# sleep3r/Diffusion-Handwriting-Generation.pytorch

Measured on AMD Instinct MI355X. Metric: stroke-points/sec reverse-sampled (T=60, L=488), higher is better.
Workload: dtype bf16; 1 GPU; configs[1]: batch=64 prompts/GPU, T=60, L=488, Lt=30, d_model=128/192/256, num_layers=2, diffusion_mode=new, random-init weights; global_batch=64, seq_len=488, parallelism=batch-shard x1 (no collectives)

## Files before the change

diffusion-handwriting-generation.pytorch_amd/csrc/dhw_api.cpp:

```cpp
#include <hip/hip_runtime.h>

#include <algorithm>
#include <cmath>
#include <cstdarg>
#include <cstdio>
#include <cstdlib>
#include <cstring>
#include <map>
#include <string>
#include <vector>

#include "../../include/dhw.h"
#include "abi_guard.h"
#include "xcd_swizzle.h"
#include "../../include/dhw_debug.h"
#include "dhw_kernels.h"
#include "persist.h"

namespace {

constexpr int SIG = 32, SIG_HID = 2048, VOCAB = 73, STYLE_CH = 256;
constexpr int SLACK_ROWS = 64;

ErrBuf g_err;
// ... 164 lines not shown

  float *sg_w1, *sg_b1, *sg_w2, *sg_b2, *in_w, *in_b, *out_w, *out_b, *pen_w, *pen_b, *emb;

  ConvBlockW enc1, enc2, enc4, dec3, dec2, dec1;
  std::vector<EncLayerW> el;
  void *w_sf1, *w_sf3, *w_q8, *w_kv8, *w_d8, *w_tf1, *w_tf3, *w_attd, *w_sk1, *w_sk2, *w_sk3;
  float *b_sf1, *b_sf3, *b_q8, *b_kv8, *b_d8, *b_tf1, *b_tf3, *b_attd, *b_sk1, *b_sk2, *b_sk3;
  int f_ts1, f_ts2, f_ts3, f_ts4;

  std::vector<Workspace> ws;
  int nstreams = 1;
  int nstreams_alloc = 1;
  hipStream_t sub_streams[MAX_STREAMS] = {};
  std::vector<TapSlot> taps;
  std::vector<std::string> el_name;
  int lpadT = 0, lpadS = 0, lpadX[3] = {0, 0, 0};

  bool prof = false;
  std::vector<std::string> prof_labels;
  std::vector<ProfRec> prof_recs;
  std::vector<ProfAgg> prof_agg;

  bool use_graph = true;
  int teach_every = 0;
  const float* teach_reset = nullptr;
  float* teach_capture = nullptr;
  bool fuse_heads = true;
  bool plane = true;
  bool fuse_up = true;
  bool chain = true;
  bool fuse = true;
  bool fuse_text = true;
  int text_pairs = 0;
  std::map<std::vector<uint64_t>, hipGraphExec_t> graphs;
  int64_t* d_text_stage = nullptr;
  float* d_style_stage = nullptr;
  float* d_out_stage = nullptr;
  float* d_noise_stage = nullptr;
  size_t noise_stage_cap = 0;
  uint64_t* d_seed = nullptr;

  bool persist = false;
  int persist_grid = 0;
  unsigned* d_step_sync = nullptr;
  size_t step_sync_words = 0;
  unsigned* h_step_err = nullptr;
  unsigned* d_step_err = nullptr;
  struct StepPlans { StepPlan* dev = nullptr; bool ok = false; };
  unsigned long long* d_step_trace = nullptr;
  std::map<std::vector<uint64_t>, StepPlans> plans;

  int last_B = 0, last_L = 0, last_Lt = 0;
};

namespace {

int fail(dhw_handle* h, int code, const char* fmt, ...) noexcept {
  va_list ap;
  va_start(ap, fmt);
  g_err.vsetf(fmt, ap);
  va_end(ap);
  if (h) h->err.set(g_err.c_str());
  return code;
}

#define DHW_GUARD(h, fn, R, ...) \
// ... 757 lines not shown
    GemmParams p = gp_base(c, c.S5, 4 * c2);
    p.seg[0] = GemmSeg{WS(c, sty_in), h->w_sf1, STYLE_CH, 1, 1};
    p.bias0 = h->b_sf1;
    p.silu_out = 1;
    p.out = WS(c, sty_h);
    run_gemm(c, "style.ffn1", p);
  }
  {
    GemmParams p = gp_base(c, c.S5, dt);
    p.seg[0] = GemmSeg{WS(c, sty_h), h->w_sf3, 4 * c2, 1, 0};
    p.bias0 = h->b_sf3;
    p.ln = 1;
    p.out = WS(c, sty_n);
    run_gemm(c, "style.ffn2_ln", p);
  }
  RUN_SMALL(c, "embed_ln", launch_embed_ln(h->prec, text, c.B * c.Lt, h->emb, dt, true_width(h, dt), VOCAB, WS(c, t_n), c.st));
}

void text_style_dynamic(Ctx& c) {
  dhw_handle* h = c.h;
  const int c2 = h->dims.c2, dt = 2 * c2;
  const float* g = c.film;
  const float* bt = c.film + h->film_tot;
  const int in_B = c.in_B ? c.in_B : c.B;
  if (h->fuse && h->fuse_text && textside_supported(h->prec, c.Lt, c.S5, dt)) {
    TextStyleParams q{};
    q.n = c.B; q.in_B = in_B; q.Lt = c.Lt; q.S5 = c.S5;
    q.sty_n = WS(c, sty_n); q.t_n = WS(c, t_n);
    q.film = c.film; q.film_bs = c.film_bs; q.film_div = c.film_div; q.film_tot = h->film_tot;
    q.f1 = h->f_ts1; q.f2 = h->f_ts2; q.f3 = h->f_ts3; q.f4 = h->f_ts4;
    q.w_q8 = h->w_q8; q.w_kv8 = h->w_kv8; q.w_d8 = h->w_d8; q.w_tf1 = h->w_tf1; q.w_tf3 = h->w_tf3;
    q.b_q8 = h->b_q8; q.b_kv8 = h->b_kv8; q.b_d8 = h->b_d8; q.b_tf1 = h->b_tf1; q.b_tf3 = h->b_tf3;
    q.text_out = TS(c, text_out);
    if (!c.err) {
      const double n = c.B, ddt = dt;
      Launch l(h, c.st, "ts.fused", n * (2.0 * c.S5 * ddt * 2 * ddt + 2.0 * c.Lt * ddt * ddt * 2 + 4.0 * c.Lt * c.S5 * ddt + 2.0 * c.Lt * ddt * 2 * ddt * 2),
               n * c.Lt * ddt * h->es + (double)in_B * (c.S5 + c.Lt) * ddt * h->es + 8.0 * ddt * ddt * h->es);
      hipError_t e = launch_text_style(h->prec, q, c.st);
      if (e != hipSuccess) c.err = fail(h, DHW_ERR_HIP, "text_style fused: %s", hipGetErrorString(e));
    }
    if (!c.planeT) tap(c, TAP_TS, TS(c, text_out), c.Lt, dt);
    for (size_t i = 0; i < h->el.size() && !c.err; ++i) {
      const EncLayerW& w = h->el[i];
      TextLayerParams t{};
      t.n = c.B; t.Lt = c.Lt; t.d = w.d;
      t.text_out = TS(c, text_out);
      t.w_td = w.w_td; t.b_td = w.b_td;
      t.film = c.film; t.film_bs = c.film_bs; t.film_div = c.film_div; t.film_tot = h->film_tot; t.f0 = w.f0;
      t.w_kv = w.w_kv1; t.b_kv = w.b_kv1; t.pb_k1 = w.pb_k1;
      t.k1 = ELT(c, (int)i, k1); t.vt1 = ELT(c, (int)i, vt1); t.lpadT = h->lpadT;
      if (c.err) break;
      t.pairs = h->text_pairs;
      const double n = c.B, dd = w.d;
      Launch l(h, c.st, "enc.text_fused", n * c.Lt * (2.0 * dt * dd + 4.0 * dd * dd), n * c.Lt * (dt + 2.0 * dd) * h->es + (dt * dd + 2.0 * dd * dd) * h->es);
      hipError_t e = launch_text_layer(h->prec, t, c.st);
      if (e != hipSuccess) c.err = fail(h, DHW_ERR_HIP, "text layer %s: %s", h->el_name[i].c_str(), hipGetErrorString(e));
    }
    return;
  }
  RUN_SMALL(c, "film.style", launch_film_apply(h->prec, WS(c, sty_n), in_B, c.B, c.S5, dt, g + h->f_ts1, bt + h->f_ts1, c.film_bs, c.film_div, TS(c, s1), c.st));
  RUN_SMALL(c, "film.text", launch_film_apply(h->prec, WS(c, t_n), in_B, c.B, c.Lt, dt, g + h->f_ts2, bt + h->f_ts2, c.film_bs, c.film_div, TS(c, t1), c.st));
  {
    GemmParams p = gp_text(c, c.Lt, dt);
    p.seg[0] = GemmSeg{TS(c, t1), h->w_q8, dt, 1, 0};
    p.bias0 = h->b_q8;
    p.out = TS(c, q8);
    run_gemm(c, "ts.q", p);
  }
  {
    GemmParams p = gp_base(c, c.S5, 2 * dt);
    p.seg[0] = GemmSeg{TS(c, s1), h->w_kv8, dt, 1, 0};
    p.bias0 = h->b_kv8;
    p.n_store = dt;
    p.out = TS(c, k8);
    p.vt = TS(c, vt8);
    p.vt_lpad = h->lpadS;
    run_gemm(c, "ts.kv", p);
  }
  {
    AttnParams a{};
    a.Q = TS(c, q8); a.ldq = dt;
    a.K = TS(c, k8); a.ldk = dt; a.koff = 0;
    a.Vt = TS(c, vt8); a.lpad = h->lpadS;
    a.out = TS(c, a8); a.ldo = dt;
    a.B = c.B; a.H = 8; a.D = dt / 8; a.Lq = c.Lt; a.Lk = c.S5;
    run_attn(c, "attn.text_style", a);
// ... 236 lines not shown
    h->dims.c2 = 192;
    h->padded = d.c2 != 192;
    h->device = device;
    h->prec = d.precision == DHW_PREC_F32 ? PREC_F32 : PREC_BF16;
    h->es = h->prec == PREC_F32 ? 4 : 2;
    h->spec = build_spec(d.num_layers, d.c1, d.c2, d.c3);
    h->pspec = build_spec(d.num_layers, d.c1, h->dims.c2, d.c3);
    for (size_t i = 0; i < h->spec.size(); ++i) h->key_index[h->spec[i].key] = (int)i;
    h->host_w.resize(h->spec.size());
    h->loaded.assign(h->spec.size(), 0);
    build_film_layout(h);
    build_names(h);
    if (hipSetDevice(device) != hipSuccess) return fail(nullptr, DHW_ERR_HIP, "hipSetDevice failed");
    {
      const char* e = getenv("DHW_STREAMS");
      if (e && atoi(e) >= 1) h->nstreams = std::min(atoi(e), MAX_STREAMS);
      h->nstreams = std::max(1, std::min(h->nstreams, d.max_B));
      h->nstreams_alloc = h->nstreams;
    }
    int rc = alloc_shared(h);
    h->ws.resize(h->nstreams);
    for (int i = 0; !rc && i < h->nstreams; ++i)
      if (!(rc = alloc_workspace(h, h->ws[i], i == 0 ? d.max_B : (d.max_B + h->nstreams - 1) / h->nstreams))) rc = verify_workspace(h, h->ws[i]);
    for (int i = 1; !rc && i < h->nstreams; ++i)
      if (hipStreamCreateWithFlags(&h->sub_streams[i], hipStreamNonBlocking) != hipSuccess) rc = fail(h, DHW_ERR_HIP, "stream create failed");
    if (const char* e = getenv("DHW_FUSE")) h->fuse = atoi(e) != 0;
    if (const char* e = getenv("DHW_PLANE")) h->plane = atoi(e) != 0;
    if (const char* e = getenv("DHW_FUSE_TEXT")) h->fuse_text = atoi(e) != 0;
    if (const char* e = getenv("DHW_FUSE_HEADS")) h->fuse_heads = atoi(e) != 0;
    if (const char* e = getenv("DHW_FUSE_UP")) h->fuse_up = atoi(e) != 0;
    if (const char* e = getenv("DHW_CHAIN")) h->chain = atoi(e) != 0;
    if (const char* e = getenv("DHW_PERSIST")) h->persist = atoi(e) != 0;
    if (const char* e = getenv("DHW_TEXT_PAIRS")) h->text_pairs = atoi(e) == 1 ? 1 : atoi(e) == 2 ? 2 : 0;
    if (h->padded) h->fuse = false;
    if (!rc && h->prec == PREC_BF16 && h->persist) {
      hipDeviceProp_t prop;
      if (hipGetDeviceProperties(&prop, device) != hipSuccess || persist_init() != hipSuccess) rc = fail(h, DHW_ERR_HIP, "persistent kernel setup failed: %s", hipGetErrorString(hipGetLastError()));
      else {
        h->persist_grid = prop.multiProcessorCount;
        if (hipHostMalloc((void**)&h->h_step_err, 64, hipHostMallocMapped) != hipSuccess || hipHostGetDevicePointer((void**)&h->d_step_err, h->h_step_err, 0) != hipSuccess)
          rc = fail(h, DHW_ERR_HIP, "host-mapped error word: %s", hipGetErrorString(hipGetLastError()));
        else *h->h_step_err = 0;
      }
    }
    if (!rc && enclayer_init() != hipSuccess) rc = fail(h, DHW_ERR_HIP, "kernel attribute setup failed: %s", hipGetErrorString(hipGetLastError()));
    if (!rc && convblock_init() != hipSuccess) rc = fail(h, DHW_ERR_HIP, "kernel attribute setup failed: %s", hipGetErrorString(hipGetLastError()));
    if (!rc && textside_init() != hipSuccess) rc = fail(h, DHW_ERR_HIP, "kernel attribute setup failed: %s", hipGetErrorString(hipGetLastError()));
    if (!rc && gemm_init() != hipSuccess) rc = fail(h, DHW_ERR_HIP, "kernel attribute setup failed: %s", hipGetErrorString(hipGetLastError()));
    if (rc) { ErrBuf keep = h->err; g_err = keep; return rc; }
    hold.p = nullptr;
    *out = h;
    return 0;
  });
}

void dhw_destroy(dhw_handle* h) {
  if (!h) return;
  try {
    destroy_impl(h);
  } catch (...) {
  }
}

}

namespace {
// ... 657 lines not shown
```

diffusion-handwriting-generation.pytorch_amd/csrc/dhw_kernels.h:

```cpp
#pragma once
#include <hip/hip_runtime.h>
#include <stdint.h>

enum { PREC_BF16 = 0, PREC_F32 = 1 };

struct GemmSeg {
  const void* A;
  const void* W;
  int C;
  int taps;
  int silu;
};

struct GemmParams {
  GemmSeg seg[2];
  int nseg;
  int B, L;
  int N;
  int n_store;
  const float* bias0;
  const float* bias1;
  const float* posb;
  int posb_cols;
  const float* gam;
// ... 117 lines not shown
hipError_t launch_randn_init(float* xt, long rows, int L, const uint64_t* seed_ptr, int sample_off, hipStream_t st, int iter = -1);
hipError_t launch_set_seed(uint64_t* seed_ptr, uint64_t seed, int64_t first_sample, hipStream_t st);
hipError_t gemm_init();

hipError_t launch_style_stem(int prec, const float* img, int B, int H, int W, const float* w, const float* bias, int Cp,
                             void* out, hipStream_t st);
hipError_t launch_style_dw(int prec, const void* in, int B, int H, int W, int stride, const float* w, const float* bias,
                           int Cp, void* out, hipStream_t st);
hipError_t launch_style_pool(int prec, const void* in, int B, int H, int W, int C, int NB, float* out, hipStream_t st);

struct TextStyleParams {
  int n;
  int in_B;
  int Lt, S5;
  const void* sty_n;
  const void* t_n;
  const float* film; long film_bs; int film_div; int film_tot;
  int f1, f2, f3, f4;
  const void *w_q8, *w_kv8, *w_d8, *w_tf1, *w_tf3;
  const float *b_q8, *b_kv8, *b_d8, *b_tf1, *b_tf3;
  void* text_out;
};
struct TextLayerParams {
  int n, Lt, d;
  const void* text_out;
  const void* w_td; const float* b_td;
  const float* film; long film_bs; int film_div; int film_tot; int f0;
  const void* w_kv; const float* b_kv;
  const float* pb_k1;
  void* k1;
  void* vt1; int lpadT;
  int pairs;
};
bool textside_supported(int prec, int Lt, int S5, int dt);
hipError_t launch_text_style(int prec, const TextStyleParams& p, hipStream_t st);
hipError_t launch_text_layer(int prec, const TextLayerParams& p, hipStream_t st);
hipError_t textside_init();

hipError_t launch_perturb(const float* x, const float* eps, const float* alphas, int B, int L, float* out, hipStream_t st);
hipError_t launch_loss(const float* eps, const float* pred, const float* pen, const float* pen_pred, const float* alphas, int B, int L,
                       float* out3, float* d_pred, float* d_pen, hipStream_t st);
hipError_t launch_sqnorm(const float* g, long n, float* out, hipStream_t st);
hipError_t launch_adam(float* p, const float* g, float* m, float* v, long n, float lr, float b1, float b2, float eps, float wd, int step,
                       const float* sqnorm, float max_norm, hipStream_t st);
hipError_t launch_film_silu_fwd(const float* u, const float* film, long film_bs, int goff, int boff, int B, int L, int C, float* a, float* h, hipStream_t st);
hipError_t launch_film_bwd(const float* d, const float* a, const float* u, const float* film, long film_bs, int goff, int B, int L, int C, int act,
                           float* du, float* dfilm, long dfilm_bs, int dgoff, int dboff, hipStream_t st);
hipError_t launch_silu_bwd_add(const float* d_sx, const float* x, long n, float* dx, hipStream_t st);
hipError_t launch_silu_fwd(const float* x, long n, float* out, hipStream_t st);
hipError_t launch_add(const float* a, const float* b, long n, float* out, hipStream_t st);
hipError_t launch_colsum(const float* dy, long rows, int C, float* db, hipStream_t st);
hipError_t launch_wgrad(const float* dy, const float* x, int B, int L, int Cout, int Cin, int taps, float* dw, hipStream_t st);
hipError_t launch_film_linear_bwd(const float* dfilm, const float* sigma, const float* wcat, int B, int cols, float* dw, float* db, float* dsigma, hipStream_t st);

struct OpGemm {
  const float* A; long sam, sak, sazo, sazi; int a_shift, a_tap_shift;
  const float* B; long sbk, sbn, sbzo, sbzi, sbt; int b_shift, b_z_shift;
  float* C; long scm, scn, sczo, sczi;
  int M, N, K, nzo, nzi, lr, taps;
  const float* bias; float alpha; int accumulate, bf16;
  const float* dsilu_of;
  float* act_out;
  const float* addend;
  float* rowsum;
  unsigned long long* stamps;
  const float* film_g = nullptr; const float* film_b = nullptr; long film_ps = 0; int film_rows = 1, film_act = 0; float* film_out = nullptr; const float* film_add = nullptr;
};
// ... 31 lines not shown
```

diffusion-handwriting-generation.pytorch_amd/csrc/textside.hip:

```cpp
#include <algorithm>
#include "enc_a_core.h"

namespace {

template <typename T, int D, int NK>
DHW_DEV void attn_once(
    const Frag<T> (&qf)[2], const char* kt, int SK, const char* vt, int SV, int Lk, f32x4 (&o)[D / 16]) {
  constexpr int DT = D / 16, NPF = (NK + 1) / 2;
  const int lane = threadIdx.x & 63, g = lane >> 4;
  const float scale = rsqrtf((float)D);
  f32x4 s[NK];
#pragma unroll
  for (int t = 0; t < NK; ++t) {
    s[t] = (f32x4){0, 0, 0, 0};
#pragma unroll
    for (int c = 0; c < 2; ++c) {
      const int d = 32 * c + 8 * g;
      const Frag<T> kf = d < D ? frag_load(reinterpret_cast<const T*>(kt + t * 16 * SK) + d) : frag_zero<T>();
      mma32(s[t], kf, qf[c]);
    }
  }
  float mx = -INFINITY;
#pragma unroll
  for (int t = 0; t < NK; ++t)
// ... 49 lines not shown
  }
};

template <typename T, int KMAX>
DHW_DEV void stage_film_384(char* dst, int S, const T* src, int rows_valid, int rows_tile, const float* gam, const float* bet, int tid) {
  static_assert(sizeof(T) == 2, "bf16 only");
  if (tid >= 480) return;
  const int cc = tid % 48, r0 = tid / 48;
  const f32x4 g0 = *reinterpret_cast<const f32x4*>(gam + cc * 8), g1 = *reinterpret_cast<const f32x4*>(gam + cc * 8 + 4);
  const f32x4 b0 = *reinterpret_cast<const f32x4*>(bet + cc * 8), b1 = *reinterpret_cast<const f32x4*>(bet + cc * 8 + 4);
  uint4 v[KMAX];
#pragma unroll
  for (int k = 0; k < KMAX; ++k) {
    const int r = r0 + 10 * k;
    v[k] = make_uint4(0, 0, 0, 0);
    if (r < rows_valid) v[k] = *reinterpret_cast<const uint4*>(src + (size_t)r * 384 + cc * 8);
  }
#pragma unroll
  for (int k = 0; k < KMAX; ++k) {
    const int r = r0 + 10 * k;
    if (r >= rows_tile) continue;
    if (r < rows_valid) {
      T* e = reinterpret_cast<T*>(&v[k]);
#pragma unroll
      for (int i = 0; i < 4; ++i) {
        e[i] = from_f<T>(to_f(e[i]) * g0[i] + b0[i]);
        e[4 + i] = from_f<T>(to_f(e[4 + i]) * g1[i] + b1[i]);
      }
    }
    *reinterpret_cast<uint4*>(dst + r * S + cc * 16) = v[k];
  }
}

template <typename T>
__global__ __launch_bounds__(512) __attribute__((amdgpu_waves_per_eu(2, 2))) void text_style_kernel(const TextStyleParams p) {
  constexpr int ES = sizeof(T), DM = 384, BM = 32, SM = 80, D = 48, KC = DM / 32;
  constexpr int NT = DM / 8 / 16, MT = BM / 16, MTS = SM / 16;
  constexpr int S = tile_stride<T>(DM), SVT = SM * ES + 16;
  extern __shared__ __attribute__((aligned(16))) char smem[];
  char* RS = smem;
  char* RV = RS + SM * S;
  char* RT = RV + DM * SVT;
  float* red = reinterpret_cast<float*>(RT + BM * S);
  const int tid = threadIdx.x, lane = tid & 63, wave = tid >> 6, l15 = lane & 15, g = lane >> 4;
  const int pair = blockIdx.x;
  const int bs = pair % p.in_B;
  const float* gam = p.film + (long)(pair / p.film_div) * p.film_bs;
  const float* bet = gam + p.film_tot;
  const int ntile0 = wave * NT, n0 = ntile0 * 16 + 4 * g;
  const size_t wlane = ((size_t)ntile0 * KC * 64 + lane) * 8;
  const T* sty = reinterpret_cast<const T*>(p.sty_n) + (size_t)bs * p.S5 * DM;
  const T* tn = reinterpret_cast<const T*>(p.t_n) + (size_t)bs * p.Lt * DM;
  const char* sop = RS + l15 * S + g * 8 * ES;
  const char* top = RT + l15 * S + g * 8 * ES;

  WRing<T, NT> ring;
#ifndef DHW_TEXT_SPREAD
#define DHW_TEXT_SPREAD 1
#endif
  constexpr bool TSPREAD = DHW_TEXT_SPREAD != 0;
  constexpr int FC = WRing<T, NT>::template fill_chunks<KC>(), FQ = (FC + 3) / 4;
  EpiParams<NT> ep;

  stage_film_384<T, 8>(RS, S, sty, p.S5, SM, gam + p.f1, bet + p.f1, tid);
  stage_film_384<T, 4>(RT, S, tn, p.Lt, BM, gam + p.f2, bet + p.f2, tid);
  ring.template fill_s<KC>(reinterpret_cast<const T*>(p.w_kv8) + (size_t)DM * DM + wlane);
  ep.load_bias(p.b_kv8 + DM, n0);
  lds_barrier();

  {
    f32x4 acc[NT][MTS];
    acc_zero(acc);
    ring.template run_s<MTS, KC>(acc, sop, S, KC);
    if constexpr (TSPREAD) ring.template fill_begin<KC>(reinterpret_cast<const T*>(p.w_kv8) + wlane);
    else ring.template fill_s<KC>(reinterpret_cast<const T*>(p.w_kv8) + wlane);
#pragma unroll
    for (int i = 0; i < NT; ++i) {
      if constexpr (TSPREAD) {
        if (i == 0) ring.template fill_range<KC, 0, FQ>();
        else if (i == 1) ring.template fill_range<KC, FQ, 2 * FQ>();
        else if (i == 2) ring.template fill_range<KC, 2 * FQ, 3 * FQ>();
      }
#pragma unroll
      for (int j = 0; j < MTS; ++j) {
        const int key = j * 16 + l15;
        const f32x4 v = acc[i][j] + ep.bias[i];
#pragma unroll
        for (int k = 0; k < 4; ++k) *reinterpret_cast<T*>(RV + (n0 + 16 * i + k) * SVT + key * ES) = from_f<T>(key < p.S5 ? v[k] : 0.f);
      }
    }
    if constexpr (TSPREAD) { static_assert(NT == 3, "three channel tiles per wave"); ring.template fill_range<KC, 3 * FQ, FC>(); }
    ep.load_bias(p.b_kv8, n0);
// ... 101 lines not shown
        else if (i == 1) ring.template fill_range<KC, FQ, 2 * FQ>();
        else if (i == 2) ring.template fill_range<KC, 2 * FQ, 3 * FQ>();
      }
#pragma unroll
      for (int j = 0; j < MT; ++j) {
        f32x4 v = acc[i][j] + ep.bias[i];
#pragma unroll
        for (int k = 0; k < 4; ++k) v[k] = silu_t<T>(v[k]);
        store4(reinterpret_cast<T*>(HID + (j * 16 + l15) * S) + n0 + 16 * i, v);
      }
    }
    if constexpr (TSPREAD) ring.template fill_range<KC, 3 * FQ, FC>();
    lds_barrier();
    ring.template run_s<MT, KC>(acc2, hop, S, KC);
    if (hh == 0) {
      ring.template fill_s<KC>(reinterpret_cast<const T*>(p.w_tf1) + (size_t)DM * DM + wlane);
      lds_barrier();
    }
  }
  ep.load(p.b_tf3, gam + p.f4, bet + p.f4, n0);
#pragma unroll
  for (int i = 0; i < NT; ++i)
#pragma unroll
    for (int j = 0; j < MT; ++j) acc2[i][j] += ep.bias[i];
  ln_rows<T, MT, NT, 8, BM>(acc2, red, wave, 0, lane, DM);
#pragma unroll
  for (int i = 0; i < NT; ++i)
#pragma unroll
    for (int j = 0; j < MT; ++j) store4(reinterpret_cast<T*>(T2 + (j * 16 + l15) * S) + n0 + 16 * i, acc2[i][j] * ep.gam[i] + ep.bet[i]);
  lds_barrier();
  tile_copy_out<T>(T2, S, reinterpret_cast<T*>(p.text_out) + (size_t)pair * p.Lt * DM, DM, p.Lt, DM, tid, 512);
}

template <typename T, int DMO, int PAIRS>
__global__ __launch_bounds__(512) __attribute__((amdgpu_waves_per_eu(4 / PAIRS, 4 / PAIRS))) void text_layer_kernel(const TextLayerParams p) {
  constexpr int OCC = 2 / PAIRS;
  constexpr int ES = sizeof(T), DI = 384, BM = 32 * PAIRS, KCI = DI / 32, KCO = DMO / 32;
  constexpr int WN = (DMO % 128 == 0) ? 8 : 6, NT = DMO / WN / 16, MT = BM / 16;
  constexpr int SI = tile_stride<T>(DI), SO = tile_stride<T>(DMO);
  extern __shared__ __attribute__((aligned(16))) char smem[];
  char* XS = smem;
  char* TL = XS + BM * SI;
  float* red = reinterpret_cast<float*>(TL + BM * SO);
  const int tid = threadIdx.x, lane = tid & 63, wave = tid >> 6, l15 = lane & 15, g = lane >> 4;
#ifndef DHW_TEXT_SPREAD
#define DHW_TEXT_SPREAD 1
#endif
  constexpr bool TSPREAD = DHW_TEXT_SPREAD != 0;
  const int pair = blockIdx.x * PAIRS;
  const int npair = min(PAIRS, p.n - pair);
  const float* gam = p.film + (long)(pair / p.film_div) * p.film_bs;
  const float* bet = gam + p.film_tot;
  const bool act = WN == 8 || wave < WN;
  const int wn = act ? wave : 0, ntile0 = wn * NT, n0 = ntile0 * 16 + 4 * g;

  WRing<T, NT, 24 / OCC> ring;
  constexpr int FCO = WRing<T, NT, 24 / OCC>::template fill_chunks<KCO>(), FQO = (FCO + 3) / 4;
  EpiParams<NT> ep;
  {
    const T* src = reinterpret_cast<const T*>(p.text_out) + (size_t)pair * p.Lt * DI;
    constexpr int cpr = DI * ES / 16, NU = BM * cpr / 512;
    static_assert(BM * cpr % 512 == 0, "staging chunks per thread");
    uint4 v[NU];
#pragma unroll
    for (int u = 0; u < NU; ++u) {
      const int id = tid + u * 512, r = id / cpr, cc = id - r * cpr, pr = r >> 5, rr = r & 31;
      const bool ok = pr < npair && rr < p.Lt;
      v[u] = *reinterpret_cast<const uint4*>(src + (ok ? (size_t)pr * p.Lt + rr : (size_t)0) * DI + cc * (16 / ES));
    }
#pragma unroll
    for (int u = 0; u < NU; ++u) {
      const int id = tid + u * 512, r = id / cpr, cc = id - r * cpr, pr = r >> 5, rr = r & 31;
      const bool ok = pr < npair && rr < p.Lt;
      T* e = reinterpret_cast<T*>(&v[u]);
#pragma unroll
      for (int i = 0; i < 16 / ES; ++i) e[i] = from_f<T>(silu_t<T>(to_f(e[i])));
      *reinterpret_cast<uint4*>(XS + r * SI + cc * 16) = ok ? v[u] : make_uint4(0, 0, 0, 0);
    }
  }
  if (act) {
    ring.template fill_s<KCI>(reinterpret_cast<const T*>(p.w_td) + ((size_t)ntile0 * KCI * 64 + lane) * 8);
    ep.load(p.b_td, gam + p.f0, bet + p.f0, n0);
  }
  lds_barrier();

  {
    f32x4 acc[NT][MT];
    acc_zero(acc);
    if (act) {
      ring.template run_s<MT, KCI>(acc, XS + l15 * SI + g * 8 * ES, SI, KCI);
      if constexpr (TSPREAD) { ring.template fill_begin<KCO>(reinterpret_cast<const T*>(p.w_kv) + ((size_t)ntile0 * KCO * 64 + lane) * 8); ring.template fill_range<KCO, 0, FQO>(); }
      else ring.template fill_s<KCO>(reinterpret_cast<const T*>(p.w_kv) + ((size_t)ntile0 * KCO * 64 + lane) * 8);
#pragma unroll
      for (int i = 0; i < NT; ++i)
#pragma unroll
        for (int j = 0; j < MT; ++j) acc[i][j] += ep.bias[i];
      if constexpr (TSPREAD) ring.template fill_range<KCO, FQO, 2 * FQO>();
    }
    if constexpr (TSPREAD) ln_rows<T, MT, NT, WN, BM>(acc, red, wn, 0, lane, DMO, act, [&]() { if (act) ring.template fill_range<KCO, 2 * FQO, 3 * FQO>(); });
    else ln_rows<T, MT, NT, WN, BM>(acc, red, wn, 0, lane, DMO, act);
    if (act) {
      if constexpr (TSPREAD) ring.template fill_range<KCO, 3 * FQO, FCO>();
#pragma unroll
      for (int i = 0; i < NT; ++i)
#pragma unroll
        for (int j = 0; j < MT; ++j) store4(reinterpret_cast<T*>(TL + (j * 16 + l15) * SO) + n0 + 16 * i, acc[i][j] * ep.gam[i] + ep.bet[i]);
    }
  }
  lds_barrier();

  auto copy_out = [&](void* base) {
#pragma unroll
    for (int pr = 0; pr < PAIRS; ++pr)
      if (pr < npair) tile_copy_out<T>(XS + pr * 32 * SO, SO, reinterpret_cast<T*>(base) + (size_t)(pair + pr) * p.Lt * DMO, DMO, p.Lt, DMO, tid, 512);
  };
  const char* lop = TL + l15 * SO + g * 8 * ES;
  {
    f32x4 acc[NT][MT];
    acc_zero(acc);
    if (act) {
      ep.load_bias(p.b_kv, n0);
      ring.template run_s<MT, KCO>(acc, lop, SO, KCO);
      if constexpr (TSPREAD) ring.template fill_begin<KCO>(reinterpret_cast<const T*>(p.w_kv) + ((size_t)(DMO / 16 + ntile0) * KCO * 64 + lane) * 8);
      else ring.template fill_s<KCO>(reinterpret_cast<const T*>(p.w_kv) + ((size_t)(DMO / 16 + ntile0) * KCO * 64 + lane) * 8);
#pragma unroll
      for (int i = 0; i < NT; ++i) {
        if constexpr (TSPREAD) { if (i == 0) ring.template fill_range<KCO, 0, 2 * FQO>(); else if (i == NT - 1) ring.template fill_range<KCO, 2 * FQO, FCO>(); }
#pragma unroll
        for (int j = 0; j < MT; ++j) {
          const int r = j * 16 + l15, rr = r & 31;
          f32x4 v = acc[i][j] + ep.bias[i];
          v += *reinterpret_cast<const f32x4*>(p.pb_k1 + (size_t)(rr < p.Lt ? rr : p.Lt - 1) * DMO + n0 + 16 * i);
          store4(reinterpret_cast<T*>(XS + r * SO) + n0 + 16 * i, v);
        }
      }
      if constexpr (TSPREAD && NT == 1) ring.template fill_range<KCO, 2 * FQO, FCO>();
    }
    lds_barrier();
    copy_out(p.k1);
  }
  {
    f32x4 acc[NT][MT];
    acc_zero(acc);
    if (act) {
      ep.load_bias(p.b_kv + DMO, n0);
      ring.template run_s<MT, KCO>(acc, lop, SO, KCO);
    }
    lds_barrier();
    if (act) {
#pragma unroll
      for (int i = 0; i < NT; ++i)
#pragma unroll
        for (int j = 0; j < MT; ++j) store4(reinterpret_cast<T*>(XS + (j * 16 + l15) * SO) + n0 + 16 * i, acc[i][j] + ep.bias[i]);
    }
    lds_barrier();
    copy_out(p.vt1);
  }
}

constexpr size_t text_style_lds() { return (size_t)80 * tile_stride<bf16_t>(384) + (size_t)384 * (80 * 2 + 16) + (size_t)32 * tile_stride<bf16_t>(384) + 2 * 8 * 32 * sizeof(float); }
template <int DMO, int PAIRS>
constexpr size_t text_layer_lds() {
  return (size_t)32 * PAIRS * tile_stride<bf16_t>(384) + (size_t)32 * PAIRS * tile_stride<bf16_t>(DMO) + 2 * 8 * 32 * PAIRS * sizeof(float);
}

}

hipError_t textside_init() {
  static_assert(text_style_lds() <= 160 * 1024, "text_style tile does not fit LDS");
  hipError_t e;
  if ((e = hipFuncSetAttribute(reinterpret_cast<const void*>(text_style_kernel<bf16_t>), hipFuncAttributeMaxDynamicSharedMemorySize, 160 * 1024)) != hipSuccess) return e;
#define DHW_TL_ATTR(D_, P_) if ((e = hipFuncSetAttribute(reinterpret_cast<const void*>(text_layer_kernel<bf16_t, D_, P_>), hipFuncAttributeMaxDynamicSharedMemorySize, 160 * 1024)) != hipSuccess) return e
  DHW_TL_ATTR(192, 1); DHW_TL_ATTR(256, 1); DHW_TL_ATTR(384, 1);
  DHW_TL_ATTR(192, 2); DHW_TL_ATTR(256, 2); DHW_TL_ATTR(384, 2);
#undef DHW_TL_ATTR
  return hipSuccess;
}

bool textside_supported(int prec, int Lt, int S5, int dt) { return prec == PREC_BF16 && Lt >= 1 && Lt <= 32 && S5 >= 1 && S5 <= 80 && dt == 384; }

hipError_t launch_text_style(int prec, const TextStyleParams& p, hipStream_t st) {
  if (!textside_supported(prec, p.Lt, p.S5, 384) || p.n < 1 || p.in_B < 1 || p.film_div < 1) return hipErrorInvalidValue;
  hipLaunchKernelGGL(text_style_kernel<bf16_t>, dim3(p.n), dim3(512), text_style_lds(), st, p);
  return hipGetLastError();
}

hipError_t launch_text_layer(int prec, const TextLayerParams& p, hipStream_t st) {
  if (prec != PREC_BF16 || p.Lt < 1 || p.Lt > 32 || p.n < 1 || p.film_div < 1 || p.lpadT < 32 || p.lpadT % 8) return hipErrorInvalidValue;
  const bool two = p.film_div % 2 == 0 && (p.pairs == 2 || (p.pairs == 0 && p.n >= 1024));
#define DHW_TL_LAUNCH(D_) \
  if (two) hipLaunchKernelGGL((text_layer_kernel<bf16_t, D_, 2>), dim3((p.n + 1) / 2), dim3(512), (text_layer_lds<D_, 2>()), st, p); \
  else hipLaunchKernelGGL((text_layer_kernel<bf16_t, D_, 1>), dim3(p.n), dim3(512), (text_layer_lds<D_, 1>()), st, p)
  switch (p.d) {
    case 192: DHW_TL_LAUNCH(192); break;
    case 256: DHW_TL_LAUNCH(256); break;
    case 384: DHW_TL_LAUNCH(384); break;
    default: return hipErrorInvalidValue;
  }
#undef DHW_TL_LAUNCH
  return hipGetLastError();
}
```

Measured before the change: 1.797 million stroke-points/s.

## Fuse text-style and all text encoder layers into one persistent text-plane kernel

Adds a single text_plane kernel that, per pair of samples, runs the text/style cross-attention body and then every encoder layer's text projection in turn. The SiLU-staged text tile stays in LDS across layers instead of being reloaded from global memory. This replaces one style launch plus one launch per encoder layer, and it cuts the round trips of text_out through HBM. In exchange it uses a grid capped at the CU count with a work loop, and it runs the style body serially for two pairs. Those choices may lower parallelism when B=64, and the extra LDS buffer may limit occupancy.

New measurement: 1.799 million stroke-points/s (median of 5 runs). About the same (+0.1%).

```diff
diff --git a/diffusion-handwriting-generation.pytorch_amd/csrc/dhw_api.cpp b/diffusion-handwriting-generation.pytorch_amd/csrc/dhw_api.cpp
--- a/diffusion-handwriting-generation.pytorch_amd/csrc/dhw_api.cpp
+++ b/diffusion-handwriting-generation.pytorch_amd/csrc/dhw_api.cpp
@@ -220,6 +220,7 @@
   bool fuse = true;
   bool fuse_text = true;
   int text_pairs = 0;
+  bool text_one = true;
   std::map<std::vector<uint64_t>, hipGraphExec_t> graphs;
   int64_t* d_text_stage = nullptr;
   float* d_style_stage = nullptr;
@@ -1043,15 +1044,7 @@
     q.w_q8 = h->w_q8; q.w_kv8 = h->w_kv8; q.w_d8 = h->w_d8; q.w_tf1 = h->w_tf1; q.w_tf3 = h->w_tf3;
     q.b_q8 = h->b_q8; q.b_kv8 = h->b_kv8; q.b_d8 = h->b_d8; q.b_tf1 = h->b_tf1; q.b_tf3 = h->b_tf3;
     q.text_out = TS(c, text_out);
-    if (!c.err) {
-      const double n = c.B, ddt = dt;
-      Launch l(h, c.st, "ts.fused", n * (2.0 * c.S5 * ddt * 2 * ddt + 2.0 * c.Lt * ddt * ddt * 2 + 4.0 * c.Lt * c.S5 * ddt + 2.0 * c.Lt * ddt * 2 * ddt * 2),
-               n * c.Lt * ddt * h->es + (double)in_B * (c.S5 + c.Lt) * ddt * h->es + 8.0 * ddt * ddt * h->es);
-      hipError_t e = launch_text_style(h->prec, q, c.st);
-      if (e != hipSuccess) c.err = fail(h, DHW_ERR_HIP, "text_style fused: %s", hipGetErrorString(e));
-    }
-    if (!c.planeT) tap(c, TAP_TS, TS(c, text_out), c.Lt, dt);
-    for (size_t i = 0; i < h->el.size() && !c.err; ++i) {
+    auto layer_params = [&](int i) {
       const EncLayerW& w = h->el[i];
       TextLayerParams t{};
       t.n = c.B; t.Lt = c.Lt; t.d = w.d;
@@ -1059,10 +1052,44 @@
       t.w_td = w.w_td; t.b_td = w.b_td;
       t.film = c.film; t.film_bs = c.film_bs; t.film_div = c.film_div; t.film_tot = h->film_tot; t.f0 = w.f0;
       t.w_kv = w.w_kv1; t.b_kv = w.b_kv1; t.pb_k1 = w.pb_k1;
-      t.k1 = ELT(c, (int)i, k1); t.vt1 = ELT(c, (int)i, vt1); t.lpadT = h->lpadT;
+      t.k1 = ELT(c, i, k1); t.vt1 = ELT(c, i, vt1); t.lpadT = h->lpadT;
+      t.pairs = h->text_pairs;
+      return t;
+    };
+    if (h->text_one && h->el.size() <= (size_t)TEXT_PLANE_MAX_LAYERS) {
+      TextPlaneParams pp{};
+      pp.ts = q;
+      pp.nl = (int)h->el.size();
+      pp.pairs = h->text_pairs;
+      for (int i = 0; i < pp.nl; ++i) pp.tl[i] = layer_params(i);
+      if (!c.err) {
+        const double n = c.B, ddt = dt;
+        double fl = n * (2.0 * c.S5 * ddt * 2 * ddt + 2.0 * c.Lt * ddt * ddt * 2 + 4.0 * c.Lt * c.S5 * ddt + 2.0 * c.Lt * ddt * 2 * ddt * 2);
+        double by = n * c.Lt * ddt * h->es + (double)in_B * (c.S5 + c.Lt) * ddt * h->es + 8.0 * ddt * ddt * h->es;
+        for (int i = 0; i < pp.nl; ++i) {
+          const double dd = pp.tl[i].d;
+          fl += n * c.Lt * (2.0 * ddt * dd + 4.0 * dd * dd);
+          by += n * c.Lt * 2.0 * dd * h->es + (ddt * dd + 2.0 * dd * dd) * h->es;
+        }
+        Launch l(h, c.st, "ts.plane", fl, by);
+        hipError_t e = launch_text_plane(h->prec, pp, c.st);
+        if (e != hipSuccess) c.err = fail(h, DHW_ERR_HIP, "text plane: %s", hipGetErrorString(e));
+      }
+      if (!c.planeT) tap(c, TAP_TS, TS(c, text_out), c.Lt, dt);
+      return;
+    }
+    if (!c.err) {
+      const double n = c.B, ddt = dt;
+      Launch l(h, c.st, "ts.fused", n * (2.0 * c.S5 * ddt * 2 * ddt + 2.0 * c.Lt * ddt * ddt * 2 + 4.0 * c.Lt * c.S5 * ddt + 2.0 * c.Lt * ddt * 2 * ddt * 2),
+               n * c.Lt * ddt * h->es + (double)in_B * (c.S5 + c.Lt) * ddt * h->es + 8.0 * ddt * ddt * h->es);
+      hipError_t e = launch_text_style(h->prec, q, c.st);
+      if (e != hipSuccess) c.err = fail(h, DHW_ERR_HIP, "text_style fused: %s", hipGetErrorString(e));
+    }
+    if (!c.planeT) tap(c, TAP_TS, TS(c, text_out), c.Lt, dt);
+    for (size_t i = 0; i < h->el.size() && !c.err; ++i) {
+      const TextLayerParams t = layer_params((int)i);
       if (c.err) break;
-      t.pairs = h->text_pairs;
-      const double n = c.B, dd = w.d;
+      const double n = c.B, dd = t.d;
       Launch l(h, c.st, "enc.text_fused", n * c.Lt * (2.0 * dt * dd + 4.0 * dd * dd), n * c.Lt * (dt + 2.0 * dd) * h->es + (dt * dd + 2.0 * dd * dd) * h->es);
       hipError_t e = launch_text_layer(h->prec, t, c.st);
       if (e != hipSuccess) c.err = fail(h, DHW_ERR_HIP, "text layer %s: %s", h->el_name[i].c_str(), hipGetErrorString(e));
@@ -1365,6 +1392,7 @@
     if (const char* e = getenv("DHW_CHAIN")) h->chain = atoi(e) != 0;
     if (const char* e = getenv("DHW_PERSIST")) h->persist = atoi(e) != 0;
     if (const char* e = getenv("DHW_TEXT_PAIRS")) h->text_pairs = atoi(e) == 1 ? 1 : atoi(e) == 2 ? 2 : 0;
+    if (const char* e = getenv("DHW_TEXT_ONE")) h->text_one = atoi(e) != 0;
     if (h->padded) h->fuse = false;
     if (!rc && h->prec == PREC_BF16 && h->persist) {
       hipDeviceProp_t prop;
diff --git a/diffusion-handwriting-generation.pytorch_amd/csrc/dhw_kernels.h b/diffusion-handwriting-generation.pytorch_amd/csrc/dhw_kernels.h
--- a/diffusion-handwriting-generation.pytorch_amd/csrc/dhw_kernels.h
+++ b/diffusion-handwriting-generation.pytorch_amd/csrc/dhw_kernels.h
@@ -173,7 +173,15 @@
   void* vt1; int lpadT;
   int pairs;
 };
+constexpr int TEXT_PLANE_MAX_LAYERS = 8;
+struct TextPlaneParams {
+  TextStyleParams ts;
+  int nl;
+  int pairs;
+  TextLayerParams tl[TEXT_PLANE_MAX_LAYERS];
+};
 bool textside_supported(int prec, int Lt, int S5, int dt);
+hipError_t launch_text_plane(int prec, const TextPlaneParams& p, hipStream_t st);
 hipError_t launch_text_style(int prec, const TextStyleParams& p, hipStream_t st);
 hipError_t launch_text_layer(int prec, const TextLayerParams& p, hipStream_t st);
 hipError_t textside_init();
diff --git a/diffusion-handwriting-generation.pytorch_amd/csrc/textside.hip b/diffusion-handwriting-generation.pytorch_amd/csrc/textside.hip
--- a/diffusion-handwriting-generation.pytorch_amd/csrc/textside.hip
+++ b/diffusion-handwriting-generation.pytorch_amd/csrc/textside.hip
@@ -105,18 +105,20 @@
   }
 }
 
+#ifndef DHW_TEXT_SPREAD
+#define DHW_TEXT_SPREAD 1
+#endif
+
 template <typename T>
-__global__ __launch_bounds__(512) __attribute__((amdgpu_waves_per_eu(2, 2))) void text_style_kernel(const TextStyleParams p) {
+DHW_DEV void text_style_body(const TextStyleParams& p, const int pair, char* smem, const int tid) {
   constexpr int ES = sizeof(T), DM = 384, BM = 32, SM = 80, D = 48, KC = DM / 32;
   constexpr int NT = DM / 8 / 16, MT = BM / 16, MTS = SM / 16;
   constexpr int S = tile_stride<T>(DM), SVT = SM * ES + 16;
-  extern __shared__ __attribute__((aligned(16))) char smem[];
   char* RS = smem;
   char* RV = RS + SM * S;
   char* RT = RV + DM * SVT;
   float* red = reinterpret_cast<float*>(RT + BM * S);
-  const int tid = threadIdx.x, lane = tid & 63, wave = tid >> 6, l15 = lane & 15, g = lane >> 4;
-  const int pair = blockIdx.x;
+  const int lane = tid & 63, wave = tid >> 6, l15 = lane & 15, g = lane >> 4;
   const int bs = pair % p.in_B;
   const float* gam = p.film + (long)(pair / p.film_div) * p.film_bs;
   const float* bet = gam + p.film_tot;
@@ -128,9 +130,6 @@
   const char* top = RT + l15 * S + g * 8 * ES;
 
   WRing<T, NT> ring;
-#ifndef DHW_TEXT_SPREAD
-#define DHW_TEXT_SPREAD 1
-#endif
   constexpr bool TSPREAD = DHW_TEXT_SPREAD != 0;
   constexpr int FC = WRing<T, NT>::template fill_chunks<KC>(), FQ = (FC + 3) / 4;
   EpiParams<NT> ep;
@@ -298,52 +297,52 @@
   tile_copy_out<T>(T2, S, reinterpret_cast<T*>(p.text_out) + (size_t)pair * p.Lt * DM, DM, p.Lt, DM, tid, 512);
 }
 
-template <typename T, int DMO, int PAIRS>
-__global__ __launch_bounds__(512) __attribute__((amdgpu_waves_per_eu(4 / PAIRS, 4 / PAIRS))) void text_layer_kernel(const TextLayerParams p) {
-  constexpr int OCC = 2 / PAIRS;
+template <typename T>
+__global__ __launch_bounds__(512) __attribute__((amdgpu_waves_per_eu(2, 2))) void text_style_kernel(const TextStyleParams p) {
+  extern __shared__ __attribute__((aligned(16))) char smem[];
+  text_style_body<T>(p, blockIdx.x, smem, threadIdx.x);
+}
+
+
+template <typename T, int PAIRS>
+DHW_DEV void stage_silu_text(const void* text_out, const int pair, const int npair, const int Lt, char* XS, const int tid) {
+  constexpr int ES = sizeof(T), DI = 384, BM = 32 * PAIRS, SI = tile_stride<T>(DI);
+  const T* src = reinterpret_cast<const T*>(text_out) + (size_t)pair * Lt * DI;
+  constexpr int cpr = DI * ES / 16, NU = BM * cpr / 512;
+  static_assert(BM * cpr % 512 == 0, "staging chunks per thread");
+  uint4 v[NU];
+#pragma unroll
+  for (int u = 0; u < NU; ++u) {
+    const int id = tid + u * 512, r = id / cpr, cc = id - r * cpr, pr = r >> 5, rr = r & 31;
+    const bool ok = pr < npair && rr < Lt;
+    v[u] = *reinterpret_cast<const uint4*>(src + (ok ? (size_t)pr * Lt + rr : (size_t)0) * DI + cc * (16 / ES));
+  }
+#pragma unroll
+  for (int u = 0; u < NU; ++u) {
+    const int id = tid + u * 512, r = id / cpr, cc = id - r * cpr, pr = r >> 5, rr = r & 31;
+    const bool ok = pr < npair && rr < Lt;
+    T* e = reinterpret_cast<T*>(&v[u]);
+#pragma unroll
+    for (int i = 0; i < 16 / ES; ++i) e[i] = from_f<T>(silu_t<T>(to_f(e[i])));
+    *reinterpret_cast<uint4*>(XS + r * SI + cc * 16) = ok ? v[u] : make_uint4(0, 0, 0, 0);
+  }
+}
+
+template <typename T, int DMO, int PAIRS, int RING>
+DHW_DEV void text_layer_body(const TextLayerParams& p, const int pair, const int npair, const char* XS, char* TL, char* KV, float* red, const int tid) {
   constexpr int ES = sizeof(T), DI = 384, BM = 32 * PAIRS, KCI = DI / 32, KCO = DMO / 32;
   constexpr int WN = (DMO % 128 == 0) ? 8 : 6, NT = DMO / WN / 16, MT = BM / 16;
   constexpr int SI = tile_stride<T>(DI), SO = tile_stride<T>(DMO);
-  extern __shared__ __attribute__((aligned(16))) char smem[];
-  char* XS = smem;
-  char* TL = XS + BM * SI;
-  float* red = reinterpret_cast<float*>(TL + BM * SO);
-  const int tid = threadIdx.x, lane = tid & 63, wave = tid >> 6, l15 = lane & 15, g = lane >> 4;
-#ifndef DHW_TEXT_SPREAD
-#define DHW_TEXT_SPREAD 1
-#endif
+  const int lane = tid & 63, wave = tid >> 6, l15 = lane & 15, g = lane >> 4;
   constexpr bool TSPREAD = DHW_TEXT_SPREAD != 0;
-  const int pair = blockIdx.x * PAIRS;
-  const int npair = min(PAIRS, p.n - pair);
   const float* gam = p.film + (long)(pair / p.film_div) * p.film_bs;
   const float* bet = gam + p.film_tot;
   const bool act = WN == 8 || wave < WN;
   const int wn = act ? wave : 0, ntile0 = wn * NT, n0 = ntile0 * 16 + 4 * g;
 
-  WRing<T, NT, 24 / OCC> ring;
-  constexpr int FCO = WRing<T, NT, 24 / OCC>::template fill_chunks<KCO>(), FQO = (FCO + 3) / 4;
+  WRing<T, NT, RING> ring;
+  constexpr int FCO = WRing<T, NT, RING>::template fill_chunks<KCO>(), FQO = (FCO + 3) / 4;
   EpiParams<NT> ep;
-  {
-    const T* src = reinterpret_cast<const T*>(p.text_out) + (size_t)pair * p.Lt * DI;
-    constexpr int cpr = DI * ES / 16, NU = BM * cpr / 512;
-    static_assert(BM * cpr % 512 == 0, "staging chunks per thread");
-    uint4 v[NU];
-#pragma unroll
-    for (int u = 0; u < NU; ++u) {
-      const int id = tid + u * 512, r = id / cpr, cc = id - r * cpr, pr = r >> 5, rr = r & 31;
-      const bool ok = pr < npair && rr < p.Lt;
-      v[u] = *reinterpret_cast<const uint4*>(src + (ok ? (size_t)pr * p.Lt + rr : (size_t)0) * DI + cc * (16 / ES));
-    }
-#pragma unroll
-    for (int u = 0; u < NU; ++u) {
-      const int id = tid + u * 512, r = id / cpr, cc = id - r * cpr, pr = r >> 5, rr = r & 31;
-      const bool ok = pr < npair && rr < p.Lt;
-      T* e = reinterpret_cast<T*>(&v[u]);
-#pragma unroll
-      for (int i = 0; i < 16 / ES; ++i) e[i] = from_f<T>(silu_t<T>(to_f(e[i])));
-      *reinterpret_cast<uint4*>(XS + r * SI + cc * 16) = ok ? v[u] : make_uint4(0, 0, 0, 0);
-    }
-  }
   if (act) {
     ring.template fill_s<KCI>(reinterpret_cast<const T*>(p.w_td) + ((size_t)ntile0 * KCI * 64 + lane) * 8);
     ep.load(p.b_td, gam + p.f0, bet + p.f0, n0);
@@ -378,7 +377,7 @@
   auto copy_out = [&](void* base) {
 #pragma unroll
     for (int pr = 0; pr < PAIRS; ++pr)
-      if (pr < npair) tile_copy_out<T>(XS + pr * 32 * SO, SO, reinterpret_cast<T*>(base) + (size_t)(pair + pr) * p.Lt * DMO, DMO, p.Lt, DMO, tid, 512);
+      if (pr < npair) tile_copy_out<T>(KV + pr * 32 * SO, SO, reinterpret_cast<T*>(base) + (size_t)(pair + pr) * p.Lt * DMO, DMO, p.Lt, DMO, tid, 512);
   };
   const char* lop = TL + l15 * SO + g * 8 * ES;
   {
@@ -397,7 +396,7 @@
           const int r = j * 16 + l15, rr = r & 31;
           f32x4 v = acc[i][j] + ep.bias[i];
           v += *reinterpret_cast<const f32x4*>(p.pb_k1 + (size_t)(rr < p.Lt ? rr : p.Lt - 1) * DMO + n0 + 16 * i);
-          store4(reinterpret_cast<T*>(XS + r * SO) + n0 + 16 * i, v);
+          store4(reinterpret_cast<T*>(KV + r * SO) + n0 + 16 * i, v);
         }
       }
       if constexpr (TSPREAD && NT == 1) ring.template fill_range<KCO, 2 * FQO, FCO>();
@@ -417,14 +416,78 @@
 #pragma unroll
       for (int i = 0; i < NT; ++i)
 #pragma unroll
-        for (int j = 0; j < MT; ++j) store4(reinterpret_cast<T*>(XS + (j * 16 + l15) * SO) + n0 + 16 * i, acc[i][j] + ep.bias[i]);
+        for (int j = 0; j < MT; ++j) store4(reinterpret_cast<T*>(KV + (j * 16 + l15) * SO) + n0 + 16 * i, acc[i][j] + ep.bias[i]);
     }
     lds_barrier();
     copy_out(p.vt1);
   }
 }
 
+template <typename T, int DMO, int PAIRS>
+__global__ __launch_bounds__(512) __attribute__((amdgpu_waves_per_eu(4 / PAIRS, 4 / PAIRS))) void text_layer_kernel(const TextLayerParams p) {
+  constexpr int BM = 32 * PAIRS, SI = tile_stride<T>(384), SO = tile_stride<T>(DMO);
+  extern __shared__ __attribute__((aligned(16))) char smem[];
+  char* XS = smem;
+  char* TL = XS + BM * SI;
+  float* red = reinterpret_cast<float*>(TL + BM * SO);
+  const int pair = blockIdx.x * PAIRS;
+  const int npair = min(PAIRS, p.n - pair);
+  stage_silu_text<T, PAIRS>(p.text_out, pair, npair, p.Lt, XS, threadIdx.x);
+  text_layer_body<T, DMO, PAIRS, 24 / (2 / PAIRS)>(p, pair, npair, XS, TL, XS, red, threadIdx.x);
+}
+
+template <typename T, int PAIRS>
+__global__ __launch_bounds__(512) __attribute__((amdgpu_waves_per_eu(2, 2))) void text_plane_kernel(const TextPlaneParams pv) {
+#ifdef __HIP_DEVICE_COMPILE__
+  const TextPlaneParams& p = *(const TextPlaneParams*)__builtin_amdgcn_kernarg_segment_ptr();
+#else
+  const TextPlaneParams& p = pv;
+#endif
+  constexpr int BM = 32 * PAIRS, S = tile_stride<T>(384);
+  extern __shared__ __attribute__((aligned(16))) char smem[];
+  char* XS = smem;
+  char* TL = XS + BM * S;
+  char* KV = TL + BM * S;
+  float* red = reinterpret_cast<float*>(KV + BM * S);
+  const int G = gridDim.x, w = blockIdx.x, n = p.ts.n;
+  const int R = PAIRS == 2 ? n / (2 * G) : 0, P0 = 2 * G * R, r = n - P0, n2 = (PAIRS == 2 && r > G) ? r - G : 0;
+  auto tid_ = []() { int t = threadIdx.x; asm volatile("" : "+v"(t)); return t & 511; };
+  for (int k = 0;; ++k) {
+    int pair, np;
+    if (k < R) pair = 2 * (w + k * G), np = 2;
+    else if (w < n2) {
+      if (k > R) break;
+      pair = P0 + 2 * w, np = 2;
+    } else {
+      const int s = w - n2 + (k - R) * G;
+      if (s >= r - 2 * n2) break;
+      pair = P0 + 2 * n2 + s, np = 1;
+    }
+    lds_barrier();
+    text_style_body<T>(p.ts, pair, smem, tid_());
+    if (PAIRS == 2 && np > 1) {
+      lds_barrier();
+      text_style_body<T>(p.ts, pair + 1, smem, tid_());
+    }
+    asm volatile("s_waitcnt vmcnt(0)" ::: "memory");
+    __syncthreads();
+    stage_silu_text<T, PAIRS>(p.ts.text_out, pair, np, p.ts.Lt, XS, tid_());
+    for (int li = 0; li < p.nl; ++li) {
+      const TextLayerParams& lp = p.tl[li];
+      switch (lp.d) {
+        case 192: text_layer_body<T, 192, PAIRS, 24>(lp, pair, np, XS, TL, KV, red, tid_()); break;
+        case 256: text_layer_body<T, 256, PAIRS, 24>(lp, pair, np, XS, TL, KV, red, tid_()); break;
+        default: text_layer_body<T, 384, PAIRS, 24>(lp, pair, np, XS, TL, KV, red, tid_()); break;
+      }
+    }
+  }
+}
+
 constexpr size_t text_style_lds() { return (size_t)80 * tile_stride<bf16_t>(384) + (size_t)384 * (80 * 2 + 16) + (size_t)32 * tile_stride<bf16_t>(384) + 2 * 8 * 32 * sizeof(float); }
+template <int PAIRS>
+constexpr size_t text_plane_lds() {
+  return std::max(text_style_lds(), (size_t)3 * 32 * PAIRS * tile_stride<bf16_t>(384) + 2 * 8 * 32 * PAIRS * sizeof(float));
+}
 template <int DMO, int PAIRS>
 constexpr size_t text_layer_lds() {
   return (size_t)32 * PAIRS * tile_stride<bf16_t>(384) + (size_t)32 * PAIRS * tile_stride<bf16_t>(DMO) + 2 * 8 * 32 * PAIRS * sizeof(float);
@@ -440,6 +503,9 @@
   DHW_TL_ATTR(192, 1); DHW_TL_ATTR(256, 1); DHW_TL_ATTR(384, 1);
   DHW_TL_ATTR(192, 2); DHW_TL_ATTR(256, 2); DHW_TL_ATTR(384, 2);
 #undef DHW_TL_ATTR
+  static_assert(text_plane_lds<2>() <= 160 * 1024, "text_plane tiles do not fit LDS");
+  if ((e = hipFuncSetAttribute(reinterpret_cast<const void*>(text_plane_kernel<bf16_t, 1>), hipFuncAttributeMaxDynamicSharedMemorySize, 160 * 1024)) != hipSuccess) return e;
+  if ((e = hipFuncSetAttribute(reinterpret_cast<const void*>(text_plane_kernel<bf16_t, 2>), hipFuncAttributeMaxDynamicSharedMemorySize, 160 * 1024)) != hipSuccess) return e;
   return hipSuccess;
 }
 
@@ -466,3 +532,24 @@
 #undef DHW_TL_LAUNCH
   return hipGetLastError();
 }
+
+hipError_t launch_text_plane(int prec, const TextPlaneParams& p, hipStream_t st) {
+  const TextStyleParams& q = p.ts;
+  if (!textside_supported(prec, q.Lt, q.S5, 384) || q.n < 1 || q.in_B < 1 || q.film_div < 1 || p.nl < 1 || p.nl > TEXT_PLANE_MAX_LAYERS) return hipErrorInvalidValue;
+  for (int i = 0; i < p.nl; ++i) {
+    const TextLayerParams& t = p.tl[i];
+    if (t.n != q.n || t.Lt != q.Lt || t.film_div != q.film_div || t.text_out != q.text_out || (t.d != 192 && t.d != 256 && t.d != 384)) return hipErrorInvalidValue;
+  }
+  static int cus = 0;
+  if (!cus) {
+    int dev = 0;
+    hipError_t e = hipGetDevice(&dev);
+    if (e == hipSuccess) e = hipDeviceGetAttribute(&cus, hipDeviceAttributeMultiprocessorCount, dev);
+    if (e != hipSuccess || cus < 1) return e != hipSuccess ? e : hipErrorInvalidValue;
+  }
+  const int G = std::min(q.n, cus);
+  const bool two = q.film_div % 2 == 0 && (p.pairs == 2 || (p.pairs == 0 && q.n > G));
+  if (two) hipLaunchKernelGGL((text_plane_kernel<bf16_t, 2>), dim3(G), dim3(512), text_plane_lds<2>(), st, p);
+  else hipLaunchKernelGGL((text_plane_kernel<bf16_t, 1>), dim3(G), dim3(512), text_plane_lds<1>(), st, p);
+  return hipGetLastError();
+}
```
